# wildltr/ptranking

Hardware: NVIDIA H100
Metric: queries/sec (LambdaRank train step, 256-doc lists) (higher is better)
Workload: dtype f32

## Files before the change

ptranking_b200/csrc/ffnet_tc.cuh:

```cuda
#pragma once
#include "common.cuh"
#include "tc.cuh"
#include "ffnet_act.cuh"

namespace ptrb200 {

struct RowsGemmArgs {
    const float* P;
    const float* scale;
    const float* shift;
    int act;
    int gr_prev;
    DropCfg drop;
    const float* P2;
    const float *kc1, *kc3, *kc0;
    int gr_cur;
    const unsigned char* b_img_hi;
    const unsigned char* b_img_lo;
    const float* bias;
    float* a_out;
    float* Out;
    double* partials;
    int rows, K, N, NP;
    int n_tile;
    int tail_off;
    int tile_rows;
    int seg_len;
    int group_rows;
    int tiles_per_group;
    int round_bf16;
};

enum { RG_FWD = 0, RG_DGRAD = 1 };

template <int ACT = -1>
static __device__ __forceinline__ float4 prologue4(const RowsGemmArgs& g, float4 v, int row, int k, bool with_dropout, size_t coef_row_off) {
    if (g.scale) {
        const size_t o = coef_row_off + k;
        const float4 sc = *reinterpret_cast<const float4*>(g.scale + o);
        const float4 sh = *reinterpret_cast<const float4*>(g.shift + o);
        v.x = fmaf(v.x, sc.x, sh.x); v.y = fmaf(v.y, sc.y, sh.y); v.z = fmaf(v.z, sc.z, sh.z); v.w = fmaf(v.w, sc.w, sh.w);
    }
    const int af = ACT >= 0 ? ACT : g.act;
    if (af != PTRB200_AF_NONE) {
        v.x = activate(af, v.x).y; v.y = activate(af, v.y).y; v.z = activate(af, v.z).y; v.w = activate(af, v.w).y;
    }
    if (with_dropout && g.drop.thr) {
        const uint64_t e = (uint64_t)row * g.K + k;
        const uint64_t d = dropout_draw4(g.drop.key, e >> 2);
        v.x = ((uint32_t)(d) & 0xffffu) >= g.drop.thr ? v.x * g.drop.scale : 0.0f;
        v.y = ((uint32_t)(d >> 16) & 0xffffu) >= g.drop.thr ? v.y * g.drop.scale : 0.0f;
        v.z = ((uint32_t)(d >> 32) & 0xffffu) >= g.drop.thr ? v.z * g.drop.scale : 0.0f;
        v.w = ((uint32_t)(d >> 48)) >= g.drop.thr ? v.w * g.drop.scale : 0.0f;
    }
    return v;
}

static __device__ __forceinline__ float bf16_rn(float x) {
    const uint32_t u = __float_as_uint(x);
    return __uint_as_float((u + 0x7fffu + ((u >> 16) & 1u)) & 0xffff0000u);
}
static __device__ __forceinline__ void store_split(unsigned char* hi, unsigned char* lo, uint32_t off, float4 v, bool split, bool to_bf16 = false, bool rn = false) {
    if (to_bf16) v = make_float4(bf16_rn(v.x), bf16_rn(v.y), bf16_rn(v.z), bf16_rn(v.w));
    if (split) {
        float4 h, l;
        if (rn) {
            tc::split_tf32_rn(v.x, h.x, l.x); tc::split_tf32_rn(v.y, h.y, l.y);
            tc::split_tf32_rn(v.z, h.z, l.z); tc::split_tf32_rn(v.w, h.w, l.w);
        } else {
            tc::split_tf32(v.x, h.x, l.x); tc::split_tf32(v.y, h.y, l.y);
            tc::split_tf32(v.z, h.z, l.z); tc::split_tf32(v.w, h.w, l.w);
        }
        *reinterpret_cast<float4*>(hi + off) = h;
        *reinterpret_cast<float4*>(lo + off) = l;
    } else {
        *reinterpret_cast<float4*>(hi + off) = v;
    }
}

static __device__ __forceinline__ float4 ldg4_guard(const float* p, int k, int K) {
    return (k < K) ? __ldg(reinterpret_cast<const float4*>(p)) : make_float4(0.f, 0.f, 0.f, 0.f);
}

static __device__ __forceinline__ float4 ldg_bf16x4(const float* base, size_t elem) {
    const uint2 u = __ldg(reinterpret_cast<const uint2*>(reinterpret_cast<const uint16_t*>(base) + elem));
    return make_float4(__uint_as_float(u.x << 16), __uint_as_float(u.x & 0xffff0000u),
                       __uint_as_float(u.y << 16), __uint_as_float(u.y & 0xffff0000u));
}
template <bool XB>
static __device__ __forceinline__ float4 ldg_a4(const float* base, size_t elem) {
    if constexpr (XB) return ldg_bf16x4(base, elem);
    else return __ldg(reinterpret_cast<const float4*>(base + elem));
}

struct PackJob {
    const float* src;
    unsigned char *img_hi, *img_lo;
    int src_cols, N, NP, K, nchunks, transpose, round_bf16;
};
constexpr int PACK_MAX_JOBS = 2 * PTRB200_MAX_FF_LAYERS;
struct PackJobs { PackJob job[PACK_MAX_JOBS]; };

__global__ void pack_b_images_kernel(const __grid_constant__ PackJobs jobs) {
    const PackJob& jb = jobs.job[blockIdx.y];
    const float* __restrict__ src = jb.src;
    unsigned char* __restrict__ img_hi = jb.img_hi;
    unsigned char* __restrict__ img_lo = jb.img_lo;
    const int src_cols = jb.src_cols, N = jb.N, NP = jb.NP, K = jb.K, nchunks = jb.nchunks;
    const bool TRANSPOSE = jb.transpose != 0;
    const int total = nchunks * NP * 8;
    for (int u = blockIdx.x * blockDim.x + threadIdx.x; u < total; u += gridDim.x * blockDim.x) {
        const int c = u / (NP * 8), rem = u % (NP * 8), r = rem >> 3, j = rem & 7, k = c * 32 + j * 4;
        float v[4] = {0.f, 0.f, 0.f, 0.f};
        if (r < N) {
#pragma unroll
            for (int e = 0; e < 4; ++e)
                if (k + e < K) v[e] = TRANSPOSE ? src[(size_t)(k + e) * src_cols + r] : src[(size_t)r * src_cols + k + e];
        }
        const size_t off = (size_t)c * NP * 128 + tc::swz_offset(r, j);
        if (jb.round_bf16) {
#pragma unroll
            for (int e = 0; e < 4; ++e) v[e] = bf16_rn(v[e]);
        }
        float4 h, l;
        tc::split_tf32_rn(v[0], h.x, l.x); tc::split_tf32_rn(v[1], h.y, l.y); tc::split_tf32_rn(v[2], h.z, l.z); tc::split_tf32_rn(v[3], h.w, l.w);
        if (img_lo) {
            *reinterpret_cast<float4*>(img_hi + off) = h;
            *reinterpret_cast<float4*>(img_lo + off) = l;
        } else {
            *reinterpret_cast<float4*>(img_hi + off) = make_float4(v[0], v[1], v[2], v[3]);
        }
    }
}

template <bool TRANSPOSE>
__global__ void pack_b_image_kernel(const float* __restrict__ src, int src_rows, int src_cols,
                                    unsigned char* __restrict__ img_hi, unsigned char* __restrict__ img_lo,
                                    int N, int NP, int K, int nchunks, int round_bf16 = 0) {
    const int total = nchunks * NP * 8;
    for (int u = blockIdx.x * blockDim.x + threadIdx.x; u < total; u += gridDim.x * blockDim.x) {
        const int c = u / (NP * 8), rem = u % (NP * 8), r = rem >> 3, j = rem & 7, k = c * 32 + j * 4;
        float v[4] = {0.f, 0.f, 0.f, 0.f};
        if (r < N) {
#pragma unroll
            for (int e = 0; e < 4; ++e)
                if (k + e < K) v[e] = TRANSPOSE ? src[(size_t)(k + e) * src_cols + r] : src[(size_t)r * src_cols + k + e];
        }
        if (round_bf16) {
#pragma unroll
            for (int e = 0; e < 4; ++e) v[e] = bf16_rn(v[e]);
        }
        const size_t off = (size_t)c * NP * 128 + tc::swz_offset(r, j);
        float4 h, l;
        tc::split_tf32_rn(v[0], h.x, l.x); tc::split_tf32_rn(v[1], h.y, l.y); tc::split_tf32_rn(v[2], h.z, l.z); tc::split_tf32_rn(v[3], h.w, l.w);
        if (img_lo) {
            *reinterpret_cast<float4*>(img_hi + off) = h;
            *reinterpret_cast<float4*>(img_lo + off) = l;
        } else {
            *reinterpret_cast<float4*>(img_hi + off) = make_float4(v[0], v[1], v[2], v[3]);
        }
    }
}

constexpr int RG_THREADS = 256;
constexpr int RG_MAX_N = 128;

template <int MODE, int PASSES, int ACT = -1, bool XB = false>
__global__ void __launch_bounds__(RG_THREADS) rows_gemm_tc_kernel(RowsGemmArgs g) {
    extern __shared__ __align__(1024) unsigned char smem_raw[];
    unsigned char* base = reinterpret_cast<unsigned char*>((reinterpret_cast<uintptr_t>(smem_raw) + 1023) & ~(uintptr_t)1023);
    const int N_full = g.N, NP_full = g.NP;
    const int n0 = blockIdx.y * g.n_tile;
    const int N = min(g.n_tile, N_full - n0);
    const int NP = ((N + 15) / 16) * 16;
    unsigned char* a_hi = base;
    unsigned char* a_lo = a_hi + 16384;
    unsigned char* b_buf = a_lo + 16384;
    const uint32_t b_stage = (uint32_t)NP * 128u * (PASSES == 3 ? 2u : 1u);
    unsigned char* tail = base + g.tail_off;
    uint64_t* bbar = reinterpret_cast<uint64_t*>(tail);
    float* otile = reinterpret_cast<float*>(base);

    const int tid = threadIdx.x, wg = tid >> 7;
    int row0, nrows, slot0;
    {
        const int t = blockIdx.x;
        if (g.group_rows > 0) {
            const int grp = t / g.tiles_per_group, tt = t % g.tiles_per_group;
            row0 = grp * g.group_rows + tt * 128;
            nrows = min(128, g.group_rows - tt * 128);
            slot0 = t;
        } else {
            row0 = t * g.tile_rows;
            nrows = min(g.tile_rows, g.rows - row0);
            slot0 = (row0 / g.seg_len);
        }
    }
    const int K = g.K;
    const int nchunks = (K + 31) / 32;
    const bool long_k = PASSES == 3 && nchunks > 5;
    if (tid == 0) { tc::mbar_init(bbar, 1); tc::mbar_init(bbar + 1, 1); tc::mbar_fence_init(); }
    __syncthreads();
    constexpr int A_UNITS = 128 * 8 / RG_THREADS;
    size_t coef_off[A_UNITS];
#pragma unroll
    for (int i = 0; i < A_UNITS; ++i) {
        const int r = (tid + i * RG_THREADS) >> 3;
        coef_off[i] = (g.scale && g.gr_prev < g.rows) ? (size_t)((row0 + min(r, nrows - 1)) / g.gr_prev) * K : 0;
    }

    float4 nav[A_UNITS];
    auto load_chunk = [&](int c) {
#pragma unroll
        for (int i = 0; i < A_UNITS; ++i) {
            const int u = tid + i * RG_THREADS, r = u >> 3, j = u & 7, k = c * 32 + j * 4;
            if constexpr (XB) nav[i] = (r < nrows && k < K) ? ldg_bf16x4(g.P, (size_t)(row0 + r) * K + k) : make_float4(0.f, 0.f, 0.f, 0.f);
            else nav[i] = (r < nrows) ? ldg4_guard(g.P + (size_t)(row0 + r) * K + k, k, K) : make_float4(0.f, 0.f, 0.f, 0.f);
        }
    };
    load_chunk(0);
    tc::with_width(NP, [&](auto W) {
    constexpr int NPc = decltype(W)::value;
    float acc[NPc / 2], acc2[NPc / 2];
#pragma unroll
    for (int e = 0; e < NPc / 2; ++e) { acc[e] = 0.0f; acc2[e] = 0.0f; }
    for (int c = 0; c < nchunks; ++c) {
        const int k0 = c * 32;
        float4 av[A_UNITS];
#pragma unroll
        for (int i = 0; i < A_UNITS; ++i) av[i] = nav[i];
        if (c + 1 < nchunks) load_chunk(c + 1);
        if (c > 0) __syncthreads();
        if (tid == 0) {
            auto fetch_b = [&](int cc) {
                const uint32_t bytes = (uint32_t)NP * 128u;
                const size_t src = ((size_t)cc * NP_full + n0) * 128u;
                unsigned char* dst = b_buf + (size_t)(cc & 1) * b_stage;
                tc::mbar_expect_tx(bbar + (cc & 1), PASSES == 3 ? 2 * bytes : bytes);
                tc::bulk_g2s(dst, g.b_img_hi + src, bytes, bbar + (cc & 1));
                if (PASSES == 3) tc::bulk_g2s(dst + bytes, g.b_img_lo + src, bytes, bbar + (cc & 1));
            };
            if (c == 0) fetch_b(0);
            if (c + 1 < nchunks) fetch_b(c + 1);
        }
#pragma unroll
        for (int i = 0; i < A_UNITS; ++i) {
            const int u = tid + i * RG_THREADS, r = u >> 3, j = u & 7, k = k0 + j * 4;
            float4 v = av[i];
            if (r < nrows && k < K) {
                if (MODE == RG_DGRAD && g.P2) {
                    const size_t kc = (g.gr_cur < g.rows ? (size_t)((row0 + r) / g.gr_cur) * K : (size_t)0) + k;
                    const float4 z = __ldg(reinterpret_cast<const float4*>(g.P2 + (size_t)(row0 + r) * K + k));
                    const float4 a1 = __ldg(reinterpret_cast<const float4*>(g.kc1 + kc));
                    const float4 a3 = __ldg(reinterpret_cast<const float4*>(g.kc3 + kc));
                    const float4 a0 = __ldg(reinterpret_cast<const float4*>(g.kc0 + kc));
                    v.x = fmaf(a1.x, v.x, fmaf(a3.x, z.x, a0.x)); v.y = fmaf(a1.y, v.y, fmaf(a3.y, z.y, a0.y));
                    v.z = fmaf(a1.z, v.z, fmaf(a3.z, z.z, a0.z)); v.w = fmaf(a1.w, v.w, fmaf(a3.w, z.w, a0.w));
                }
                v = prologue4<ACT>(g, v, row0 + r, k, MODE == RG_FWD, coef_off[i]);
                if (MODE == RG_FWD && g.a_out && blockIdx.y == 0) *reinterpret_cast<float4*>(g.a_out + (size_t)(row0 + r) * K + k) = v;
            } else v = make_float4(0.f, 0.f, 0.f, 0.f);
            store_split(a_hi, a_lo, tc::swz_offset(r, j), v, PASSES == 3, PASSES == 1 && g.round_bf16 != 0, long_k);
        }
        tc::fence_proxy_async();
        __syncthreads();
        tc::mbar_wait(bbar + (c & 1), (c >> 1) & 1);
        const uint32_t a_s = tc::smem_u32(a_hi) + wg * 8192;
        const uint32_t b_hi_s = tc::smem_u32(b_buf) + (uint32_t)(c & 1) * b_stage, b_lo_s = b_hi_s + (uint32_t)NP * 128u;
        tc::wg_fence();
#pragma unroll
        for (int s = 0; s < 4; ++s) {
            const uint64_t ah = tc::smem_desc_sw128(a_s + s * 32, 1024);
            const uint64_t bh = tc::smem_desc_sw128(b_hi_s + s * 32, 1024);
            if (PASSES == 3) {
                const uint64_t al = tc::smem_desc_sw128(a_s + 16384 + s * 32, 1024);
                const uint64_t bl = tc::smem_desc_sw128(b_lo_s + s * 32, 1024);
                tc::mma_tf32<NPc>(acc2, al, bh, 1u);
                tc::mma_tf32<NPc>(acc2, ah, bl, 1u);
            }
            tc::mma_tf32<NPc>(acc, ah, bh, 1u);
        }
        tc::wg_commit();
        tc::wg_wait<0>();
    }
    __syncthreads();

#pragma unroll
    for (int e = 0; e < NPc / 2; ++e) {
        const int r = wg * 64 + tc::acc_row(e), col = tc::acc_col(e);
        if (col >= N) continue;
        float v = PASSES == 3 ? acc[e] + acc2[e] : acc[e];
        if (MODE == RG_FWD) v += __ldg(g.bias + n0 + col);
        else if (g.drop.thr)
            v = dropout_keep(g.drop.key, (uint64_t)(row0 + r) * N_full + n0 + col, g.drop.thr) ? v * g.drop.scale : 0.0f;
        otile[(size_t)r * N + col] = v;
    }
    });
    __syncthreads();
    if (N == N_full) {
        const size_t total = (size_t)nrows * N;
        float* dst = g.Out + (size_t)row0 * N;
        if ((N & 3) == 0) {
            const float4* s4 = reinterpret_cast<const float4*>(otile);
            float4* d4 = reinterpret_cast<float4*>(dst);
            for (size_t i = tid; i < total / 4; i += RG_THREADS) d4[i] = s4[i];
        } else {
            for (size_t i = tid; i < total; i += RG_THREADS) dst[i] = otile[i];
        }
    } else {
        const int q4 = N >> 2;
        for (int i = tid; i < nrows * q4; i += RG_THREADS) {
            const int r = i / q4, qq = i - r * q4;
            *reinterpret_cast<float4*>(g.Out + (size_t)(row0 + r) * N_full + n0 + qq * 4) = *reinterpret_cast<const float4*>(otile + (size_t)r * N + qq * 4);
        }
    }
    if (MODE == RG_FWD && g.partials) {
        for (int cidx = tid; cidx < N; cidx += RG_THREADS) {
            int seg = 0;
            for (int rbeg = 0; rbeg < nrows; rbeg += g.seg_len, ++seg) {
                const int rend = min(nrows, rbeg + g.seg_len);
                double s1 = 0.0, s2 = 0.0;
                for (int r = rbeg; r < rend; ++r) {
                    const float z = otile[(size_t)r * N + cidx];
                    s1 += (double)z; s2 += (double)z * (double)z;
                }
                double* p = g.partials + ((size_t)(slot0 + seg) * N_full + n0 + cidx) * 2;
                p[0] = s1; p[1] = s2;
            }
        }
    }
}

constexpr int RW_EPI_WARPS = 8, RW_PROD_WARPS = 8;
constexpr int RW_THREADS = (RW_EPI_WARPS + RW_PROD_WARPS) * 32;
constexpr int RW_PRODUCERS = RW_PROD_WARPS * 32;
constexpr int RW_PU = 128 * 8 / RW_PRODUCERS;
constexpr int RW_MAX_N = 128;
constexpr int RW_CONS_REGS = 120, RW_PROD_REGS = 136;
static_assert((RW_CONS_REGS * RW_EPI_WARPS + RW_PROD_REGS * RW_PROD_WARPS) * 32 <= 65536, "register split exceeds the register file");

struct RowsWsExtra {
    int ntiles;
    int stats_mode;
    int nchunks;
};

static __device__ __forceinline__ void rw_tile(const RowsGemmArgs& g, int t, int& row0, int& nrows) {
    if (g.group_rows > 0) {
        const int grp = t / g.tiles_per_group, tt = t - grp * g.tiles_per_group;
        row0 = grp * g.group_rows + tt * 128;
        nrows = min(128, g.group_rows - tt * 128);
    } else {
        row0 = t * g.tile_rows;
        nrows = min(g.tile_rows, g.rows - row0);
    }
}

template <int MODE, int PASSES, int ACT, int KT = 0, bool XB = false>
__global__ void __launch_bounds__(RW_THREADS, 1) rows_gemm_ws_kernel(RowsGemmArgs g, RowsWsExtra x) {
    extern __shared__ __align__(1024) unsigned char smem_raw[];
    unsigned char* base = reinterpret_cast<unsigned char*>((reinterpret_cast<uintptr_t>(smem_raw) + 1023) & ~(uintptr_t)1023);
    const int NP = g.NP, K = KT ? KT : g.K, N = g.N, nchunks = KT ? (KT + 31) / 32 : x.nchunks;
    const int wchunk = NP * 128;
    unsigned char* w_hi = base;
    unsigned char* w_lo = w_hi + (size_t)nchunks * wchunk;
    unsigned char* a_ring = w_lo + (PASSES == 3 ? (size_t)nchunks * wchunk : 0);
    float* stat_sm = reinterpret_cast<float*>(a_ring + 2 * 32768);
    uint64_t* bars = reinterpret_cast<uint64_t*>(stat_sm + RW_EPI_WARPS * NP * 2);
    uint64_t* wfull = bars;
    uint64_t* aready = bars + 1;
    uint64_t* afree = bars + 3;

    const int tid = threadIdx.x, warp = tid >> 5, lane = tid & 31;
    if (tid == 0) {
        tc::mbar_init(wfull, 1);
        for (int i = 0; i < 2; ++i) { tc::mbar_init(aready + i, RW_PROD_WARPS); tc::mbar_init(afree + i, RW_EPI_WARPS); }
        tc::mbar_fence_init();
    }
    __syncthreads();
    const int my_tiles = blockIdx.x < x.ntiles ? (x.ntiles - blockIdx.x + gridDim.x - 1) / gridDim.x : 0;

    if (warp >= RW_EPI_WARPS) {
        tc::setmaxnreg_inc<RW_PROD_REGS>();
        if constexpr (MODE == RG_DGRAD) {
            const int ptid = tid - RW_EPI_WARPS * 32;
            const int j4 = (ptid & 7) * 4;
            int r_[RW_PU];
            uint32_t sw_[RW_PU];
    #pragma unroll
            for (int i = 0; i < RW_PU; ++i) { r_[i] = (ptid >> 3) + i * (RW_PRODUCERS / 8); sw_[i] = tc::swz_offset(r_[i], ptid & 7); }
            const int total_q = my_tiles * nchunks;
            const bool has_coef = g.scale != nullptr;
            const bool per_group = has_coef && g.gr_prev < g.rows;
            const bool fused_dz = MODE == RG_DGRAD && g.P2 != nullptr;
            float4 pre[RW_PU], pre2[RW_PU];
            size_t soff[RW_PU];
            bool ok[RW_PU];
            auto point = [&](int it) {
                int r0, nr;
                rw_tile(g, blockIdx.x + it * gridDim.x, r0, nr);
    #pragma unroll
                for (int i = 0; i < RW_PU; ++i) { ok[i] = r_[i] < nr; soff[i] = (size_t)(r0 + min(r_[i], nr - 1)) * K + j4; }
            };
            auto fetch = [&](int c) {
                const bool kv = c * 32 + j4 < K;
    #pragma unroll
                for (int i = 0; i < RW_PU; ++i) {
                    pre[i] = (ok[i] && kv) ? __ldg(reinterpret_cast<const float4*>(g.P + soff[i] + c * 32)) : make_float4(0.f, 0.f, 0.f, 0.f);
                    if (MODE == RG_DGRAD) pre2[i] = (fused_dz && ok[i] && kv) ? __ldg(reinterpret_cast<const float4*>(g.P2 + soff[i] + c * 32)) : make_float4(0.f, 0.f, 0.f, 0.f);
                }
            };
            if (total_q > 0) { point(0); fetch(0); }
            int q = 0;
            for (int it = 0; it < my_tiles; ++it) {
                int row0, nrows;
                rw_tile(g, blockIdx.x + it * gridDim.x, row0, nrows);
                bool live[RW_PU];
                float* aout[RW_PU];
                const float* sc[RW_PU];
                const float* sh[RW_PU];
                size_t kco[RW_PU];
                uint64_t dq[RW_PU];
    #pragma unroll
                for (int i = 0; i < RW_PU; ++i) {
                    live[i] = r_[i] < nrows;
                    const size_t e0 = (size_t)(row0 + min(r_[i], nrows - 1)) * K + j4;
                    aout[i] = (MODE == RG_FWD && g.a_out) ? g.a_out + e0 : nullptr;
                    const size_t co = per_group ? (size_t)((row0 + min(r_[i], nrows - 1)) / g.gr_prev) * K + j4 : (size_t)j4;
                    sc[i] = has_coef ? g.scale + co : nullptr;
                    sh[i] = has_coef ? g.shift + co : nullptr;
                    kco[i] = (fused_dz && g.gr_cur < g.rows) ? (size_t)((row0 + min(r_[i], nrows - 1)) / g.gr_cur) * K + j4 : (size_t)j4;
                    dq[i] = (uint64_t)e0 >> 2;
                }
    #pragma unroll 1
            for (int c = 0; c < nchunks; ++c, ++q) {
                    const int s = q & 1;
                    float4 cur[RW_PU], cur2[RW_PU];
    #pragma unroll
                    for (int i = 0; i < RW_PU; ++i) { cur[i] = pre[i]; cur2[i] = pre2[i]; }
                    if (q + 1 < total_q) {
                        if (c + 1 < nchunks) fetch(c + 1); else { point(it + 1); fetch(0); }
                    }
                    if (q >= 2) tc::mbar_wait(afree + s, ((q - 2) >> 1) & 1);
                    unsigned char* a_hi = a_ring + s * 32768;
                    const bool kv = c * 32 + j4 < K;
    #pragma unroll
                    for (int i = 0; i < RW_PU; ++i) {
                        float4 v = cur[i];
                        if (live[i] && kv) {
                            if (MODE == RG_DGRAD && fused_dz) {
                                const float4 a1 = __ldg(reinterpret_cast<const float4*>(g.kc1 + kco[i] + c * 32));
                                const float4 a3 = __ldg(reinterpret_cast<const float4*>(g.kc3 + kco[i] + c * 32));
                                const float4 a0 = __ldg(reinterpret_cast<const float4*>(g.kc0 + kco[i] + c * 32));
                                const float4 z = cur2[i];
                                v.x = fmaf(a1.x, v.x, fmaf(a3.x, z.x, a0.x)); v.y = fmaf(a1.y, v.y, fmaf(a3.y, z.y, a0.y));
                                v.z = fmaf(a1.z, v.z, fmaf(a3.z, z.z, a0.z)); v.w = fmaf(a1.w, v.w, fmaf(a3.w, z.w, a0.w));
                            }
                            if (has_coef) {
                                const float4 a = __ldg(reinterpret_cast<const float4*>(sc[i] + c * 32));
                                const float4 b = __ldg(reinterpret_cast<const float4*>(sh[i] + c * 32));
                                v.x = fmaf(v.x, a.x, b.x); v.y = fmaf(v.y, a.y, b.y); v.z = fmaf(v.z, a.z, b.z); v.w = fmaf(v.w, a.w, b.w);
                            }
                            if (ACT != PTRB200_AF_NONE) {
                                const int af = ACT < 0 ? g.act : ACT;
                                v.x = activate(af, v.x).y; v.y = activate(af, v.y).y; v.z = activate(af, v.z).y; v.w = activate(af, v.w).y;
                            }
                            if (MODE == RG_FWD && g.drop.thr) {
                                const uint64_t d = dropout_draw4(g.drop.key, dq[i] + c * 8);
                                v.x = ((uint32_t)(d) & 0xffffu) >= g.drop.thr ? v.x * g.drop.scale : 0.0f;
                                v.y = ((uint32_t)(d >> 16) & 0xffffu) >= g.drop.thr ? v.y * g.drop.scale : 0.0f;
                                v.z = ((uint32_t)(d >> 32) & 0xffffu) >= g.drop.thr ? v.z * g.drop.scale : 0.0f;
                                v.w = ((uint32_t)(d >> 48)) >= g.drop.thr ? v.w * g.drop.scale : 0.0f;
                            }
                            if (MODE == RG_FWD && aout[i]) *reinterpret_cast<float4*>(aout[i] + c * 32) = v;
                        } else v = make_float4(0.f, 0.f, 0.f, 0.f);
                        store_split(a_hi, a_hi + 16384, sw_[i], v, PASSES == 3, PASSES == 1 && g.round_bf16 != 0);
                    }
                    tc::fence_proxy_async();
                    __syncwarp();
                    if (lane == 0) tc::mbar_arrive(aready + s);
                }
            }
        } else {
            const int ptid = tid - RW_EPI_WARPS * 32;
            const int j4 = (ptid & 7) * 4;
            int r_[RW_PU];
            uint32_t sw_[RW_PU];
    #pragma unroll
            for (int i = 0; i < RW_PU; ++i) { r_[i] = (ptid >> 3) + i * (RW_PRODUCERS / 8); sw_[i] = tc::swz_offset(r_[i], ptid & 7); }
            const int total_q = my_tiles * nchunks;
            const bool has_coef = g.scale != nullptr;
            const bool per_group = has_coef && g.gr_prev < g.rows;
            const bool fused_dz = MODE == RG_DGRAD && g.P2 != nullptr;
            const int lastc = nchunks - 1;
            const int vlast = (K - lastc * 32 + 3) >> 2;
            const bool partial = MODE == RG_FWD && vlast < 8;
            const int zfill = 8;
            const int rB = ptid & 127;
            int jB_[RW_PU];
    #pragma unroll
            for (int i = 0; i < RW_PU; ++i) jB_[i] = (ptid >> 7) + i * (RW_PRODUCERS / 128);
            float4 pre[RW_PU], pre2[RW_PU];
            size_t soff[RW_PU], soffB[RW_PU];
            bool ok[RW_PU], okB[RW_PU];
            auto point = [&](int it) {
                int r0, nr;
                rw_tile(g, blockIdx.x + it * gridDim.x, r0, nr);
    #pragma unroll
                for (int i = 0; i < RW_PU; ++i) {
                    ok[i] = r_[i] < nr; soff[i] = (size_t)(r0 + min(r_[i], nr - 1)) * K + j4;
                    okB[i] = rB < nr && jB_[i] < vlast; soffB[i] = (size_t)(r0 + min(rB, nr - 1)) * K + lastc * 32 + min(jB_[i], vlast - 1) * 4;
                }
            };
            auto fetch = [&](int c) {
                if (partial && c == lastc) {
    #pragma unroll
                    for (int i = 0; i < RW_PU; ++i) {
                        pre[i] = okB[i] ? ldg_a4<XB>(g.P, soffB[i]) : make_float4(0.f, 0.f, 0.f, 0.f);
                        if (MODE == RG_DGRAD) pre2[i] = (fused_dz && okB[i]) ? __ldg(reinterpret_cast<const float4*>(g.P2 + soffB[i])) : make_float4(0.f, 0.f, 0.f, 0.f);
                    }
                    return;
                }
                const bool kv = c * 32 + j4 < K;
    #pragma unroll
                for (int i = 0; i < RW_PU; ++i) {
                    pre[i] = (ok[i] && kv) ? ldg_a4<XB>(g.P, soff[i] + c * 32) : make_float4(0.f, 0.f, 0.f, 0.f);
                    if (MODE == RG_DGRAD) pre2[i] = (fused_dz && ok[i] && kv) ? __ldg(reinterpret_cast<const float4*>(g.P2 + soff[i] + c * 32)) : make_float4(0.f, 0.f, 0.f, 0.f);
                }
            };
            auto xform = [&](float4 v, const float4 z, const float* scp, const float* shp, size_t kcoff, uint64_t dquad, float* aoutp) -> float4 {
                if (MODE == RG_DGRAD && fused_dz) {
                    const float4 a1 = __ldg(reinterpret_cast<const float4*>(g.kc1 + kcoff));
                    const float4 a3 = __ldg(reinterpret_cast<const float4*>(g.kc3 + kcoff));
                    const float4 a0 = __ldg(reinterpret_cast<const float4*>(g.kc0 + kcoff));
                    v.x = fmaf(a1.x, v.x, fmaf(a3.x, z.x, a0.x)); v.y = fmaf(a1.y, v.y, fmaf(a3.y, z.y, a0.y));
                    v.z = fmaf(a1.z, v.z, fmaf(a3.z, z.z, a0.z)); v.w = fmaf(a1.w, v.w, fmaf(a3.w, z.w, a0.w));
                }
                if (has_coef) {
                    const float4 a = __ldg(reinterpret_cast<const float4*>(scp));
                    const float4 b = __ldg(reinterpret_cast<const float4*>(shp));
                    v.x = fmaf(v.x, a.x, b.x); v.y = fmaf(v.y, a.y, b.y); v.z = fmaf(v.z, a.z, b.z); v.w = fmaf(v.w, a.w, b.w);
                }
                if (ACT != PTRB200_AF_NONE) {
                    const int af = ACT < 0 ? g.act : ACT;
                    v.x = activate(af, v.x).y; v.y = activate(af, v.y).y; v.z = activate(af, v.z).y; v.w = activate(af, v.w).y;
                }
                if (MODE == RG_FWD && g.drop.thr) {
                    const uint64_t d = dropout_draw4(g.drop.key, dquad);
                    v.x = ((uint32_t)(d) & 0xffffu) >= g.drop.thr ? v.x * g.drop.scale : 0.0f;
                    v.y = ((uint32_t)(d >> 16) & 0xffffu) >= g.drop.thr ? v.y * g.drop.scale : 0.0f;
                    v.z = ((uint32_t)(d >> 32) & 0xffffu) >= g.drop.thr ? v.z * g.drop.scale : 0.0f;
                    v.w = ((uint32_t)(d >> 48)) >= g.drop.thr ? v.w * g.drop.scale : 0.0f;
                }
                if (MODE == RG_FWD && aoutp) *reinterpret_cast<float4*>(aoutp) = v;
                return v;
            };
            if (total_q > 0) { point(0); fetch(0); }
            int q = 0;
            for (int it = 0; it < my_tiles; ++it) {
                int row0, nrows;
                rw_tile(g, blockIdx.x + it * gridDim.x, row0, nrows);
                bool live[RW_PU];
                float* aout[RW_PU];
                const float* sc[RW_PU];
                const float* sh[RW_PU];
                size_t kco[RW_PU];
                uint64_t dq[RW_PU];
    #pragma unroll
                for (int i = 0; i < RW_PU; ++i) {
                    live[i] = r_[i] < nrows;
                    const size_t e0 = (size_t)(row0 + min(r_[i], nrows - 1)) * K + j4;
                    aout[i] = (MODE == RG_FWD && g.a_out) ? g.a_out + e0 : nullptr;
                    const size_t co = per_group ? (size_t)((row0 + min(r_[i], nrows - 1)) / g.gr_prev) * K + j4 : (size_t)j4;
                    sc[i] = has_coef ? g.scale + co : nullptr;
                    sh[i] = has_coef ? g.shift + co : nullptr;
                    kco[i] = (fused_dz && g.gr_cur < g.rows) ? (size_t)((row0 + min(r_[i], nrows - 1)) / g.gr_cur) * K + j4 : (size_t)j4;
                    dq[i] = (uint64_t)e0 >> 2;
                }
    #pragma unroll (KT ? 8 : 1)
            for (int c = 0; c < nchunks; ++c, ++q) {
                    const int s = q & 1;
                    float4 cur[RW_PU], cur2[RW_PU];
    #pragma unroll
                    for (int i = 0; i < RW_PU; ++i) { cur[i] = pre[i]; cur2[i] = pre2[i]; }
                    if (q + 1 < total_q) {
                        if (c + 1 < nchunks) fetch(c + 1); else { point(it + 1); fetch(0); }
                    }
                    if (q >= 2) tc::mbar_wait(afree + s, ((q - 2) >> 1) & 1);
                    unsigned char* a_hi = a_ring + s * 32768;
                    if (partial && c == lastc) {
    #pragma unroll
                        for (int i = 0; i < RW_PU; ++i) {
                            const int jB = jB_[i];
                            if (jB < zfill) {
                                float4 v = make_float4(0.f, 0.f, 0.f, 0.f);
                                if (jB < vlast && rB < nrows) {
                                    const int col = lastc * 32 + jB * 4;
                                    const size_t e0 = (size_t)(row0 + rB) * K + col;
                                    const size_t co = (per_group ? (size_t)((row0 + rB) / g.gr_prev) * K : (size_t)0) + col;
                                    const size_t kc = ((fused_dz && g.gr_cur < g.rows) ? (size_t)((row0 + rB) / g.gr_cur) * K : (size_t)0) + col;
                                    v = xform(cur[i], cur2[i], has_coef ? g.scale + co : nullptr, has_coef ? g.shift + co : nullptr, kc,
                                              (uint64_t)e0 >> 2, (MODE == RG_FWD && g.a_out) ? g.a_out + e0 : nullptr);
                                }
                                store_split(a_hi, a_hi + 16384, tc::swz_offset(rB, jB), v, PASSES == 3, PASSES == 1 && g.round_bf16 != 0);
                            }
                        }
                    } else {
                        const bool kv = c * 32 + j4 < K;
    #pragma unroll
                        for (int i = 0; i < RW_PU; ++i) {
                            float4 v = make_float4(0.f, 0.f, 0.f, 0.f);
                            if (live[i] && kv)
                                v = xform(cur[i], cur2[i], has_coef ? sc[i] + c * 32 : nullptr, has_coef ? sh[i] + c * 32 : nullptr,
                                          kco[i] + c * 32, dq[i] + c * 8, aout[i] ? aout[i] + c * 32 : nullptr);
                            store_split(a_hi, a_hi + 16384, sw_[i], v, PASSES == 3, PASSES == 1 && g.round_bf16 != 0);
                        }
                    }
                    tc::fence_proxy_async();
                    __syncwarp();
                    if (lane == 0) tc::mbar_arrive(aready + s);
                }
            }
        }
    } else {
        tc::setmaxnreg_dec<RW_CONS_REGS>();
        if (my_tiles > 0) {
        const int wg = warp >> 2;
        if (tid == 0) {
            tc::mbar_expect_tx(wfull, (uint32_t)(nchunks * wchunk * (PASSES == 3 ? 2 : 1)));
            for (int c = 0; c < nchunks; ++c) {
                tc::bulk_g2s(w_hi + (size_t)c * wchunk, g.b_img_hi + (size_t)c * wchunk, wchunk, wfull);
                if (PASSES == 3) tc::bulk_g2s(w_lo + (size_t)c * wchunk, g.b_img_lo + (size_t)c * wchunk, wchunk, wfull);
            }
        }
        tc::mbar_wait(wfull, 0);
        const uint32_t a_base = tc::smem_u32(a_ring) + wg * 8192, wh_base = tc::smem_u32(w_hi), wl_base = tc::smem_u32(w_lo);
        double acc1 = 0.0, acc2 = 0.0;
        tc::with_width(NP, [&](auto W) {
        constexpr int NPc = decltype(W)::value;
        int q = 0;
        for (int it = 0; it < my_tiles; ++it) {
            const int t = blockIdx.x + it * gridDim.x;
            int row0, nrows;
            rw_tile(g, t, row0, nrows);
            float acc[NPc / 2];
#pragma unroll
            for (int e = 0; e < NPc / 2; ++e) acc[e] = 0.0f;
    #pragma unroll (KT ? 8 : 1)
            for (int c = 0; c < nchunks; ++c, ++q) {
                const int s = q & 1;
                tc::mbar_wait(aready + s, (q >> 1) & 1);
                uint32_t a_addr = a_base + s * 32768, b_off = c * wchunk;
                asm volatile("" : "+r"(a_addr), "+r"(b_off));
                const uint64_t ah = tc::smem_desc_sw128(a_addr, 1024), al = tc::smem_desc_sw128(a_addr + 16384, 1024);
                const uint64_t bh = tc::smem_desc_sw128(wh_base + b_off, 1024), bl = tc::smem_desc_sw128(wl_base + b_off, 1024);
                tc::wg_fence();
#pragma unroll
                for (int st = 0; st < 4; ++st) {
                    if (PASSES == 3) {
                        tc::mma_tf32<NPc>(acc, al + 2 * st, bh + 2 * st, 1u);
                        tc::mma_tf32<NPc>(acc, ah + 2 * st, bl + 2 * st, 1u);
                    }
                    tc::mma_tf32<NPc>(acc, ah + 2 * st, bh + 2 * st, 1u);
                }
                tc::wg_commit();
                tc::wg_wait<1>();
                if (c > 0) { __syncwarp(); if (lane == 0) tc::mbar_arrive(afree + (s ^ 1)); }
            }
            tc::wg_wait<0>();
            __syncwarp();
            if (lane == 0) tc::mbar_arrive(afree + ((q - 1) & 1));
            const float* bias = g.bias;
            asm volatile("" : "+l"(bias));
            bool live[2];
            float* orow[2];
#pragma unroll
            for (int h = 0; h < 2; ++h) {
                const int r = wg * 64 + tc::acc_row(2 * h);
                live[h] = r < nrows;
                orow[h] = g.Out + (size_t)(row0 + min(r, nrows - 1)) * N;
            }
#pragma unroll
            for (int e = 0; e < NPc / 2; ++e) {
                const int col = tc::acc_col(e);
                if (col >= N) { acc[e] = 0.0f; continue; }
                if (MODE == RG_FWD) acc[e] += __ldg(bias + col);
                else if (g.drop.thr) {
                    const int r = wg * 64 + tc::acc_row(e);
                    acc[e] = dropout_keep(g.drop.key, (uint64_t)(row0 + r) * N + col, g.drop.thr) ? acc[e] * g.drop.scale : 0.0f;
                }
            }
#pragma unroll
            for (int e = 0; e < NPc / 2; e += 2) {
                const int col = tc::acc_col(e), h = (e >> 1) & 1;
                if (!live[h] || col >= N) continue;
                if ((N & 1) == 0) *reinterpret_cast<float2*>(orow[h] + col) = make_float2(acc[e], acc[e + 1]);
                else { orow[h][col] = acc[e]; if (col + 1 < N) orow[h][col + 1] = acc[e + 1]; }
            }
            if (MODE == RG_FWD && x.stats_mode) {
                int sl = lane, sw = warp;
                asm volatile("" : "+r"(sl), "+r"(sw));
#pragma unroll
                for (int j = 0; j < NPc / 16; ++j) {
                    const float* w = acc + 8 * j;
                    float s1[4], s2[4];
#pragma unroll
                    for (int p = 0; p < 4; ++p) {
                        const int e0 = (p >> 1) * 4 + (p & 1), e1 = e0 + 2;
                        const float v0 = live[0] ? w[e0] : 0.0f, v1 = live[1] ? w[e1] : 0.0f;
                        s1[p] = v0 + v1; s2[p] = v0 * v0 + v1 * v1;
                    }
#pragma unroll
                    for (int p = 0; p < 4; ++p)
#pragma unroll
                        for (int o = 4; o < 32; o <<= 1) {
                            s1[p] += __shfl_xor_sync(0xffffffffu, s1[p], o);
                            s2[p] += __shfl_xor_sync(0xffffffffu, s2[p], o);
                        }
                    if (sl < 4) {
#pragma unroll
                        for (int p = 0; p < 4; ++p) {
                            const int col = j * 16 + (p >> 1) * 8 + 2 * sl + (p & 1);
                            stat_sm[(sw * NP + col) * 2] = s1[p];
                            stat_sm[(sw * NP + col) * 2 + 1] = s2[p];
                        }
                    }
                }
                asm volatile("bar.sync 2, 256;" ::: "memory");
                if (tid < N) {
                    double s1 = 0.0, s2 = 0.0;
#pragma unroll
                    for (int w = 0; w < RW_EPI_WARPS; ++w) { s1 += (double)stat_sm[(w * NP + tid) * 2]; s2 += (double)stat_sm[(w * NP + tid) * 2 + 1]; }
                    if (x.stats_mode == 2) {
                        double* p = g.partials + ((size_t)t * N + tid) * 2;
                        p[0] = s1; p[1] = s2;
                    } else { acc1 += s1; acc2 += s2; }
                }
                asm volatile("bar.sync 2, 256;" ::: "memory");
            }
        }
        });
        if (MODE == RG_FWD && x.stats_mode == 1 && tid < N) {
            double* p = g.partials + ((size_t)blockIdx.x * N + tid) * 2;
            p[0] = acc1; p[1] = acc2;
        }
        } else if (MODE == RG_FWD && x.stats_mode == 1 && tid < N) {
            double* p = g.partials + ((size_t)blockIdx.x * N + tid) * 2;
            p[0] = 0.0; p[1] = 0.0;
        }
    }
}

struct WgradArgs {
    const float* Z2;
    const float *kc1, *kc3, *kc0;
    int gr_cur;
    const float* dZ;
    const float* P;
    const float* scale;
    const float* shift;
    int act, gr_prev;
    DropCfg drop;
    float* partials;
    int rows, K, N;
    int KP;
    int N_full, K_full;
    int kb;
    int tile_rows;
    int stages;
    int round_bf16;
};

constexpr int WG_THREADS = 512;
constexpr int WG_MAX_STAGES = 4;

template <int PASSES, bool XB = false>
__global__ void __launch_bounds__(WG_THREADS, 1) wgrad_tc_kernel(WgradArgs g) {
    extern __shared__ __align__(1024) unsigned char smem_raw[];
    unsigned char* base = reinterpret_cast<unsigned char*>((reinterpret_cast<uintptr_t>(smem_raw) + 1023) & ~(uintptr_t)1023);
    const int R = g.tile_rows;
    const int m0 = blockIdx.y * 128, kk0 = blockIdx.z * g.kb;
    const int N = min(128, g.N_full - m0), K = min(g.kb, g.K_full - kk0), KP = ((K + 15) / 16) * 16;
    const int Nmax = min(128, g.N_full), Kmax = min(g.kb, g.K_full);
    const bool blocked = gridDim.y > 1 || gridDim.z > 1;
    const int KPmax = ((Kmax + 15) / 16) * 16;
    const int zop_bytes = 128 * 128, pop_bytes = KPmax * 128;
    const int op_bytes = (zop_bytes + pop_bytes) * (PASSES == 3 ? 2 : 1);
    const bool fused_dz = g.Z2 != nullptr;
    const int rawz1 = ((R * Nmax * 4 + 127) / 128) * 128;
    constexpr int PB = XB ? 2 : 4;
    const int rawz_bytes = rawz1 * (fused_dz ? 2 : 1), rawp_bytes = ((R * Kmax * PB + 127) / 128) * 128;
    const int stages = g.stages;
    unsigned char* opbuf = base;
    unsigned char* rawbuf = opbuf + 2 * op_bytes;
    unsigned char* tail = rawbuf + stages * (rawz_bytes + rawp_bytes);
    uint64_t* full = reinterpret_cast<uint64_t*>(tail);

    const int tid = threadIdx.x, warp = tid >> 5, lane = tid & 31, wg = warp >> 2;
    if (tid == 0) {
        for (int s = 0; s < stages; ++s) tc::mbar_init(full + s, 1);
        tc::mbar_fence_init();
    }
    const int ntiles = (g.rows + R - 1) / R;
    const int my_tiles = blockIdx.x < ntiles ? (ntiles - blockIdx.x + gridDim.x - 1) / gridDim.x : 0;

    bool p_bulk_ok = true;
    if constexpr (XB) p_bulk_ok = ((reinterpret_cast<uintptr_t>(g.P) & 15) == 0) && (!blocked || (K % 8 == 0 && g.K_full % 8 == 0));
    auto p_bulk = [&](int nrows) -> bool {
        if constexpr (XB) return p_bulk_ok && (blocked || (((uint32_t)nrows * K * 2) & 15) == 0);
        else return true;
    };

    auto issue_load = [&](int it, int s) {
        const int t = blockIdx.x + it * gridDim.x;
        const int row0 = t * R, nrows = min(R, g.rows - row0);
        const bool pbk = p_bulk(nrows);
        const uint32_t zb = (uint32_t)nrows * N * 4, pb = pbk ? (uint32_t)nrows * K * PB : 0u;
        unsigned char* rz = rawbuf + s * (rawz_bytes + rawp_bytes);
        if (!blocked) {
            if (lane == 0) {
                if ((zb & 15) == 0) {
                    tc::mbar_expect_tx(full + s, (fused_dz ? 2 * zb : zb) + pb);
                    tc::bulk_g2s(rz, g.dZ + (size_t)row0 * N, zb, full + s);
                    if (fused_dz) tc::bulk_g2s(rz + rawz1, g.Z2 + (size_t)row0 * N, zb, full + s);
                } else {
                    tc::mbar_expect_tx(full + s, pb);
                }
                if constexpr (XB) { if (pbk) tc::bulk_g2s(rz + rawz_bytes, reinterpret_cast<const uint16_t*>(g.P) + (size_t)row0 * K, pb, full + s); }
                else tc::bulk_g2s(rz + rawz_bytes, g.P + (size_t)row0 * K, pb, full + s);
            }
        } else {
            const bool z_bulk = (N & 3) == 0;
            if (lane == 0) tc::mbar_expect_tx(full + s, (z_bulk ? zb : 0u) + pb);
            __syncwarp();
            if (lane < nrows) {
                if (z_bulk) tc::bulk_g2s(rz + (size_t)lane * N * 4, g.dZ + (size_t)(row0 + lane) * g.N_full + m0, (uint32_t)N * 4, full + s);
                if constexpr (XB) {
                    if (pbk) tc::bulk_g2s(rz + rawz_bytes + (size_t)lane * K * 2, reinterpret_cast<const uint16_t*>(g.P) + (size_t)(row0 + lane) * g.K_full + kk0,
                                          (uint32_t)K * 2, full + s);
                } else tc::bulk_g2s(rz + rawz_bytes + (size_t)lane * K * 4, g.P + (size_t)(row0 + lane) * g.K_full + kk0, (uint32_t)K * 4, full + s);
            }
            __syncwarp();
        }
    };

    const bool plain_p = !g.scale && g.act == PTRB200_AF_NONE && !g.drop.thr;
    const bool single_group = fused_dz && g.gr_cur >= g.rows;
    float* coef = reinterpret_cast<float*>(tail + 128);
    {
        const uint32_t op_s = tc::smem_u32(opbuf);
        for (int e = tid; e < 2 * op_bytes / 16; e += WG_THREADS) tc::sts128(op_s + (uint32_t)e * 16u, make_float4(0.f, 0.f, 0.f, 0.f));
        if (single_group)
            for (int e = tid; e < 3 * 128; e += WG_THREADS) {
                const int which = e >> 7, n = e & 127;
                const float* src = which == 0 ? g.kc1 : which == 1 ? g.kc3 : g.kc0;
                coef[e] = n < N ? __ldg(src + m0 + n) : 0.0f;
            }
        __syncthreads();
    }
    if (warp == 0)
        for (int it = 0; it < min(stages, my_tiles); ++it) issue_load(it, it);

    auto put = [&](unsigned char* hi, unsigned char* lo, uint32_t off, float4 v) {
        if (PASSES == 3) {
            float4 h, l;
            tc::split_tf32(v.x, h.x, l.x); tc::split_tf32(v.y, h.y, l.y); tc::split_tf32(v.z, h.z, l.z); tc::split_tf32(v.w, h.w, l.w);
            *reinterpret_cast<float4*>(hi + off) = h;
            *reinterpret_cast<float4*>(lo + off) = l;
        } else {
            if (g.round_bf16) v = make_float4(bf16_rn(v.x), bf16_rn(v.y), bf16_rn(v.z), bf16_rn(v.w));
            *reinterpret_cast<float4*>(hi + off) = v;
        }
    };
    const int mh = wg & 1, KPh = ((KP / 16 + 1) / 2) * 16, c0 = (wg >> 1) ? KP - KPh : 0, cw0 = (wg >> 1) ? KPh : 0;
    const int RQ = R / 4;

    tc::with_width(KPh, [&](auto W) {
    constexpr int NPc = decltype(W)::value;
    float acc[NPc / 2];
#pragma unroll
    for (int e = 0; e < NPc / 2; ++e) acc[e] = 0.0f;
    for (int it = 0; it < my_tiles; ++it) {
        const int t = blockIdx.x + it * gridDim.x, o = it & 1, s = it % stages;
        const int row0 = t * R, nrows = min(R, g.rows - row0);
        const float* rz = reinterpret_cast<const float*>(rawbuf + s * (rawz_bytes + rawp_bytes));
        const float* rp = reinterpret_cast<const float*>(rawbuf + s * (rawz_bytes + rawp_bytes) + rawz_bytes);
        if (blocked ? (N & 3) != 0 : (((uint32_t)nrows * N * 4) & 15) != 0) {
            float* rzw = const_cast<float*>(rz);
            for (int e = tid; e < nrows * N; e += WG_THREADS) rzw[e] = g.dZ[(size_t)(row0 + e / N) * g.N_full + m0 + e % N];
            __syncthreads();
        }
        if constexpr (XB) {
            if (!p_bulk(nrows)) {
                uint16_t* rpw = reinterpret_cast<uint16_t*>(rawbuf + s * (rawz_bytes + rawp_bytes) + rawz_bytes);
                const uint16_t* src = reinterpret_cast<const uint16_t*>(g.P);
                for (int e = tid; e < nrows * K; e += WG_THREADS) rpw[e] = src[(size_t)(row0 + e / K) * g.K_full + kk0 + e % K];
                __syncthreads();
            }
        }
        tc::mbar_wait(full + s, (it / stages) & 1);
        unsigned char* zh = opbuf + o * op_bytes;
        unsigned char* zl = zh + zop_bytes;
        unsigned char* ph = zh + (PASSES == 3 ? 2 : 1) * zop_bytes;
        unsigned char* pl = ph + pop_bytes;
        for (int u = tid; u < 128 * RQ; u += WG_THREADS) {
            const int n = u & 127, qq = u >> 7;
            if (n >= N) continue;
            float v[4];
            const size_t grp_off_base = (size_t)m0 + n;
#pragma unroll
            for (int e = 0; e < 4; ++e) {
                const int r = qq * 4 + e;
                float x = 0.0f;
                if (r < nrows) {
                    x = rz[r * N + n];
                    if (fused_dz) {
                        const float z = rz[rawz1 / 4 + r * N + n];
                        float a1, a3, a0;
                        if (single_group) { a1 = coef[n]; a3 = coef[128 + n]; a0 = coef[256 + n]; }
                        else {
                            const size_t go = (size_t)((row0 + r) / g.gr_cur) * g.N_full + grp_off_base;
                            a1 = __ldg(g.kc1 + go); a3 = __ldg(g.kc3 + go); a0 = __ldg(g.kc0 + go);
                        }
                        x = fmaf(a1, x, fmaf(a3, z, a0));
                    }
                }
                v[e] = x;
            }
            put(zh, zl, tc::swz_offset(n, qq), make_float4(v[0], v[1], v[2], v[3]));
        }
        for (int u = tid; u < KP * RQ; u += WG_THREADS) {
            const int k = u % KP, qq = u / KP;
            if (k >= K) continue;
            float v[4];
#pragma unroll
            for (int e = 0; e < 4; ++e) {
                const int r = qq * 4 + e;
                float x = 0.0f;
                if (r < nrows) {
                    if constexpr (XB) x = __uint_as_float((uint32_t)reinterpret_cast<const uint16_t*>(rp)[r * K + k] << 16);
                    else x = rp[r * K + k];
                    if (!plain_p) {
                        const int row = row0 + r, col = kk0 + k;
                        if (g.scale) {
                            const size_t co = (g.gr_prev < g.rows ? (size_t)(row / g.gr_prev) * g.K_full : 0) + col;
                            x = fmaf(x, __ldg(g.scale + co), __ldg(g.shift + co));
                        }
                        if (g.act != PTRB200_AF_NONE) x = activate(g.act, x).y;
                        if (g.drop.thr) x = dropout_keep(g.drop.key, (uint64_t)row * g.K_full + col, g.drop.thr) ? x * g.drop.scale : 0.0f;
                    }
                }
                v[e] = x;
            }
            put(ph, pl, tc::swz_offset(k, qq), make_float4(v[0], v[1], v[2], v[3]));
        }
        tc::fence_proxy_async();
        __syncthreads();
        if (warp == 0 && it + stages < my_tiles) issue_load(it + stages, s);
        const uint32_t a_s = tc::smem_u32(zh) + mh * 8192, b_s = tc::smem_u32(ph) + c0 * 128;
        const uint64_t ah = tc::smem_desc_sw128(a_s, 1024), bh = tc::smem_desc_sw128(b_s, 1024);
        const uint64_t al = tc::smem_desc_sw128(a_s + zop_bytes, 1024), bl = tc::smem_desc_sw128(b_s + pop_bytes, 1024);
        tc::wg_fence();
#pragma unroll
        for (int st = 0; st < 4; ++st) {
            if (PASSES == 3) {
                tc::mma_tf32<NPc>(acc, al + 2 * st, bh + 2 * st, 1u);
                tc::mma_tf32<NPc>(acc, ah + 2 * st, bl + 2 * st, 1u);
            }
            tc::mma_tf32<NPc>(acc, ah + 2 * st, bh + 2 * st, 1u);
        }
        tc::wg_commit();
        tc::wg_wait<0>();
    }
    float* dst = g.partials + (size_t)blockIdx.x * g.N_full * g.K_full + (size_t)m0 * g.K_full + kk0;
#pragma unroll
    for (int e = 0; e < NPc / 2; ++e) {
        const int n = mh * 64 + tc::acc_row(e), k = c0 + tc::acc_col(e);
        if (n < N && k >= cw0 && k < K) dst[(size_t)n * g.K_full + k] = acc[e];
    }
    });
}

}
```

Measured before the change: 220,200.

## Vectorize dropout draws per quad and use transpose-reduce for column stats

In the backward epilogue, dropout masks are now generated with one 64-bit draw per group of four columns, shared between lane pairs via a shuffle, instead of one hash per element. This requires N divisible by 4 and otherwise falls back to the old per-element path. The forward column-statistics reduction switches from eight independent butterfly reductions to a recursive-halving transpose reduction, which cuts the number of shuffles and lets every lane write one result. The dropout change assumes dropout_draw4 yields the same mask bits as dropout_keep, otherwise masks may differ from other kernels.

```diff
diff --git a/ptranking_b200/csrc/ffnet_tc.cuh b/ptranking_b200/csrc/ffnet_tc.cuh
--- a/ptranking_b200/csrc/ffnet_tc.cuh
+++ b/ptranking_b200/csrc/ffnet_tc.cuh
@@ -680,14 +680,38 @@
                 live[h] = r < nrows;
                 orow[h] = g.Out + (size_t)(row0 + min(r, nrows - 1)) * N;
             }
-#pragma unroll
-            for (int e = 0; e < NPc / 2; ++e) {
-                const int col = tc::acc_col(e);
-                if (col >= N) { acc[e] = 0.0f; continue; }
-                if (MODE == RG_FWD) acc[e] += __ldg(bias + col);
-                else if (g.drop.thr) {
-                    const int r = wg * 64 + tc::acc_row(e);
-                    acc[e] = dropout_keep(g.drop.key, (uint64_t)(row0 + r) * N + col, g.drop.thr) ? acc[e] * g.drop.scale : 0.0f;
+            if (MODE == RG_FWD) {
+#pragma unroll
+                for (int e = 0; e < NPc / 2; ++e) {
+                    const int col = tc::acc_col(e);
+                    if (col >= N) { acc[e] = 0.0f; continue; }
+                    acc[e] += __ldg(bias + col);
+                }
+            } else if (g.drop.thr && (N & 3) == 0) {
+                const bool odd = lane & 1;
+#pragma unroll
+                for (int e = 0; e < NPc / 2; e += 4) {
+                    const int col = tc::acc_col(e);
+                    const uint64_t el = (uint64_t)(row0 + wg * 64 + tc::acc_row(e) + (odd ? 8 : 0)) * N + (col & ~3);
+                    const uint64_t d = dropout_draw4(g.drop.key, el >> 2);
+                    const uint32_t other = __shfl_xor_sync(0xffffffffu, odd ? (uint32_t)d : (uint32_t)(d >> 32), 1);
+                    const uint32_t ur = odd ? other : (uint32_t)d;
+                    const uint32_t ur8 = odd ? (uint32_t)(d >> 32) : other;
+                    if (col >= N) { acc[e] = acc[e + 1] = acc[e + 2] = acc[e + 3] = 0.0f; continue; }
+                    acc[e] = (ur & 0xffffu) >= g.drop.thr ? acc[e] * g.drop.scale : 0.0f;
+                    acc[e + 1] = (ur >> 16) >= g.drop.thr ? acc[e + 1] * g.drop.scale : 0.0f;
+                    acc[e + 2] = (ur8 & 0xffffu) >= g.drop.thr ? acc[e + 2] * g.drop.scale : 0.0f;
+                    acc[e + 3] = (ur8 >> 16) >= g.drop.thr ? acc[e + 3] * g.drop.scale : 0.0f;
+                }
+            } else {
+#pragma unroll
+                for (int e = 0; e < NPc / 2; ++e) {
+                    const int col = tc::acc_col(e);
+                    if (col >= N) { acc[e] = 0.0f; continue; }
+                    if (g.drop.thr) {
+                        const int r = wg * 64 + tc::acc_row(e);
+                        acc[e] = dropout_keep(g.drop.key, (uint64_t)(row0 + r) * N + col, g.drop.thr) ? acc[e] * g.drop.scale : 0.0f;
+                    }
                 }
             }
 #pragma unroll
@@ -703,28 +727,27 @@
 #pragma unroll
                 for (int j = 0; j < NPc / 16; ++j) {
                     const float* w = acc + 8 * j;
-                    float s1[4], s2[4];
+                    float s[8];
 #pragma unroll
                     for (int p = 0; p < 4; ++p) {
                         const int e0 = (p >> 1) * 4 + (p & 1), e1 = e0 + 2;
                         const float v0 = live[0] ? w[e0] : 0.0f, v1 = live[1] ? w[e1] : 0.0f;
-                        s1[p] = v0 + v1; s2[p] = v0 * v0 + v1 * v1;
+                        s[p] = v0 + v1; s[4 + p] = v0 * v0 + v1 * v1;
                     }
 #pragma unroll
-                    for (int p = 0; p < 4; ++p)
-#pragma unroll
-                        for (int o = 4; o < 32; o <<= 1) {
-                            s1[p] += __shfl_xor_sync(0xffffffffu, s1[p], o);
-                            s2[p] += __shfl_xor_sync(0xffffffffu, s2[p], o);
-                        }
-                    if (sl < 4) {
-#pragma unroll
-                        for (int p = 0; p < 4; ++p) {
-                            const int col = j * 16 + (p >> 1) * 8 + 2 * sl + (p & 1);
-                            stat_sm[(sw * NP + col) * 2] = s1[p];
-                            stat_sm[(sw * NP + col) * 2 + 1] = s2[p];
+                    for (int st = 0; st < 3; ++st) {
+                        const int h = 4 >> st, o = 4 << st;
+                        const bool up = sl & o;
+#pragma unroll
+                        for (int i = 0; i < h; ++i) {
+                            float keep = s[i], send = s[i + h];
+                            if (up) { const float t = keep; keep = send; send = t; }
+                            s[i] = keep + __shfl_xor_sync(0xffffffffu, send, o);
                         }
                     }
+                    const int v = ((sl >> 2) & 1) * 4 + ((sl >> 3) & 1) * 2 + ((sl >> 4) & 1), p = v & 3;
+                    const int col = j * 16 + (p >> 1) * 8 + 2 * (sl & 3) + (p & 1);
+                    stat_sm[(sw * NP + col) * 2 + (v >> 2)] = s[0];
                 }
                 asm volatile("bar.sync 2, 256;" ::: "memory");
                 if (tid < N) {
```

Result: faster. 236,800 (median of 6 runs) (+7.5%).
